# supersimple33/aruco-slam

Hardware: AMD Instinct MI355X
Metric: EKF updates/sec at n=1024 landmarks, m=32 obs/frame (higher is better)
Workload: dtype f32 covariance / f64 state

## Files before the change

aruco_slam_amd/csrc/ekf_api.hip:

```cpp
#include <atomic>
#include <cstring>

#include "ekf_host.h"
#include "ekf_kernels.h"

thread_local std::string g_err;

namespace {

std::atomic<ekf_filter*> g_pipelining{nullptr};

void release_pipelining_token(ekf_filter* f) { (void)g_pipelining.compare_exchange_strong(f, nullptr); }

constexpr int kStageSlots = 64;
constexpr int kMacroSuper = 8;
constexpr int kMacroMinTiles = 3000;
constexpr int kTimedKernels = 4;
constexpr int kWideVisible = 1024;
inline int visible_cap(int model) { return model == EKF_MODEL_ROTATIONS ? 50 : 64; }
inline bool wide_frame(int model, int m) { return m > visible_cap(model); }
constexpr int kEventPool = 2048;

struct Layout {
    int64_t cap;
// ... 39 lines not shown
    L.has_cov2 = c.cov_kernel != EKF_COVK_VALU && (c.flags & 5) == 0;
    L.off_cov2 = L.has_cov2 ? w.take((size_t)L.cap * L.cap * L.elem) : 0;
    L.off_wdbg = w.take((size_t)L.kmax * L.cap * 8);
    L.off_idx = w.take((size_t)c.max_visible * 4);
    L.off_z = w.take((size_t)c.max_visible * 7 * 8);
    L.off_status = w.take(256);
    L.off_stamps = w.take(64 * 8);
    L.off_dx = w.take((size_t)L.cap * 8);
    L.off_diag = w.take((size_t)L.cap * 8);
    L.off_xyz = w.take((size_t)256 * 6 * 8);
    L.off_unc = w.take((size_t)256 * 10 * 8);
    {
        const size_t nb = (size_t)L.kmax / EKF_RB;
        L.xl_dop = nb * (nb - 1) / 2 * 256 + 64;
        L.xl_y = L.xl_dop + nb * 256;
        L.xl_jac = L.xl_y + L.kmax;
        L.xl_tag = L.xl_jac + (size_t)L.kmax * EKF_JLD;
        L.xl_xs = L.xl_tag + 32;
        L.xl_xr = L.xl_xs + nb * (nb + 1) / 2 * 256;
        L.xl_stag = L.xl_xr + (size_t)round_up(L.kmax, 16);
        L.xl_len = L.xl_stag + 256;
        L.off_xl = w.take(2 * L.xl_len * 8);
        L.off_done = w.take(256);
        L.off_sync = w.take(256);
        L.wsup_ld = (int)round_up(EKF_CAM + (int64_t)L.lmd * c.max_visible, 32);
        L.off_wsup = w.take((size_t)2 * L.kmax * L.wsup_ld * L.elem);
    }
    {
        const int tmax = (int)(L.cap / 128);
        L.tiles_cap = (L.elem == 4 && c.cov_kernel != EKF_COVK_VALU && c.cov_kernel != EKF_COVK_MFMA_TILE)
                          ? tmax * (tmax + 1) / 2 + 8 * kMacroSuper * kMacroSuper : 0;
        L.off_tiles = w.take((size_t)L.tiles_cap * 4);
    }
    L.off_wwork = wide ? w.take((size_t)L.kmax * L.cap * 8) : 0;
    L.off_xinv = wide ? w.take((size_t)EKF_WIDE_BLOCK * EKF_WIDE_BLOCK * 8) : 0;
    L.total = w.end;
    L.slot_bytes = std::max(align256((size_t)c.max_visible * 4) + align256((size_t)c.max_visible * 56),
                            align256(256 * 48) + align256(256 * 80));
    return L;
}

int check_config(const ekf_config* c) {
    if (!c) return fail(EKF_ERR_INVALID, "config is NULL");
    if (c->max_landmarks < 1) return fail(EKF_ERR_INVALID, "max_landmarks must be >= 1");
    if (c->model != EKF_MODEL_EKF && c->model != EKF_MODEL_ROTATIONS)
        return fail(EKF_ERR_INVALID, "unknown model");
    if (c->max_visible < 1 || c->max_visible > ((c->flags & EKF_FLAG_WIDE_FRAMES) ? kWideVisible : visible_cap(c->model)))
// ... 109 lines not shown
    fr.idx = idx_dev;
    fr.z = z_dev;
    fr.jac = f->at<double>(L.off_jac);
    fr.resid = f->at<double>(L.off_resid);
    fr.lmcol = f->at<int32_t>(L.off_lmcol);
    fr.amat = f->at<double>(L.off_amat);
    fr.lda = L.cap;
    fr.sblk = f->at<double>(L.off_sblk);
    fr.sblk_rows = L.kmax;
    fr.lmat = f->at<double>(L.off_lmat);
    fr.ldl = L.kmax;
    fr.dinv = f->at<double>(L.off_dinv);
    fr.lop = f->at<double>(L.off_lop);
    fr.dop = f->at<double>(L.off_dop);
    fr.yvec = f->at<double>(L.off_y);
    fr.wpanel = f->at<void>(L.off_wpanel);
    fr.ldw = L.cap;
    fr.wdbg = f->debug_w ? f->at<double>(L.off_wdbg) : nullptr;
    fr.status = f->at<int32_t>(L.off_status);
    fr.traj_row = traj_row;
    fr.dxvec = f->at<double>(L.off_dx);
    fr.stamps = (f->debug_w || f->debug_stamps) ? f->at<long long>(L.off_stamps) : nullptr;
    fr.stamps_heavy = f->debug_stamps_light ? 0 : 1;
    fr.nz = EkfNoise{f->cfg.q_cam, f->cfg.q_err, f->cfg.q_lm, f->cfg.r_uncertainty};
    fr.quat_mode = f->cfg.quat_mode;
    fr.n_lm = f->n_lm;
    fr.state_host = nullptr;
    fr.status_host = nullptr;
    fr.cov_tiles = nullptr;
    fr.cov_grid = 0;
    if (f->tiles_T > 0 && f->tiles_T == (fr.dims + 127) / 128) {
        fr.cov_tiles = f->at<uint32_t>(L.off_tiles);
        fr.cov_grid = f->tiles_grid;
    }
    return fr;
}

bool use_front_kernel(const ekf_filter* f, const EkfFrame& fr) { return (f->cfg.flags & 4) == 0 && fr.kpad <= 192; }

void bind_exchange(ekf_filter* f, EkfFrame& fr) {
    const Layout& L = f->lay;
    double* base = f->at<double>(L.off_xl);
    fr.xl = base + (f->fseq & 1) * L.xl_len;
    fr.xl_next = base + ((f->fseq + 1) & 1) * L.xl_len;
    fr.xl_dop = (int32_t)L.xl_dop;
    fr.xl_y = (int32_t)L.xl_y;
// ... 237 lines not shown
            fr.wprev = wbuf[par ^ 1];
            fr.wsup_prev = wsup[par ^ 1];
        }
        const int nb = fr.kpad / EKF_RB;
        const int grid = nb * (nb + 1) / 2 + 2 + fr.ncols / 64;
        fr.wsup_ld = L.wsup_ld;
        fr.la_sync = sync;
        fr.la_signal = (t > 0) ? base + (uint64_t)t : 0;
        fr.la_gate = (t > 0) ? base + (uint64_t)t : 0;
        fr.lds_min = grid <= 100 ? 148 * 1024 : 0;
        if (t + 1 < frames) {
            nx = frame_at(t + 1);
            fr.next_idx = nx.idx;
            fr.next_m = nx.m;
            fr.wsup = wsup[par];
        }
        bind_exchange(f, fr);
        by_cov_type(f, [&](auto elem) { ekf_launch_front<decltype(elem)>(fr, f->stream); });
        EkfFrame cu = fr;
        cu.cov = cbuf[par];
        cu.cov_out = cbuf[par ^ 1];
        if (t + 1 < frames) {
            ekf_launch_gate(sync, base + (uint64_t)t + 1, status, f->big);
            by_cov_type(f, [&](auto elem) { ekf_launch_cov_update<decltype(elem)>(cu, 2, f->big); });
            ekf_launch_signal(sync + 1, base + (uint64_t)t + 1, f->big);
        } else {
            by_cov_type(f, [&](auto elem) { ekf_launch_cov_update<decltype(elem)>(cu, 2, f->stream); });
        }
        HIP_TRY(hipGetLastError());
        f->last_m = cf_t.m;
    }
    f->cov = cbuf[frames & 1];
    f->la_base = base + (uint64_t)frames;
    return EKF_OK;
}

struct RunPlan {
    std::vector<char> candidate;
    std::vector<char> joins;
    bool want_runs = false;
};

template <class MOf, class NNewOf>
RunPlan plan_runs(const ekf_filter* f, int frames, MOf m_of, NNewOf nnew_of) {
    RunPlan p;
    p.candidate.assign((size_t)frames, 0);
    p.joins.assign((size_t)frames, 0);
    int prev_kpad = -1;
// ... 689 lines not shown
            if (count < (size_t)kp * kp) return fail(EKF_ERR_INVALID, "out too small");
            HIP_TRY(hipMemcpy2D(out, (size_t)kp * 8, f->at<double>(L.off_lmat), (size_t)L.kmax * 8,
                                (size_t)kp * 8, kp, hipMemcpyDeviceToHost));
            return EKF_OK;
        case 3:
            if (!f->debug_w) return fail(EKF_ERR_STATE, "call ekf_debug_fetch(f,-1,..) first");
            if (count < (size_t)kp * dims) return fail(EKF_ERR_INVALID, "out too small");
            HIP_TRY(hipMemcpy2D(out, (size_t)dims * 8, f->at<double>(L.off_wdbg), (size_t)L.cap * 8,
                                (size_t)dims * 8, kp, hipMemcpyDeviceToHost));
            return EKF_OK;
        case 4:
            if (count < (size_t)k * dims) return fail(EKF_ERR_INVALID, "out too small");
            HIP_TRY(hipMemcpy2D(out, (size_t)dims * 8, f->at<double>(L.off_amat), (size_t)L.cap * 8,
                                (size_t)dims * 8, k, hipMemcpyDeviceToHost));
            return EKF_OK;
        case 5:
            if (count < 64) return fail(EKF_ERR_INVALID, "out too small");
            {
                long long st[64];
                HIP_TRY(hipMemcpy(st, f->at<long long>(L.off_stamps), sizeof(st), hipMemcpyDeviceToHost));
                for (int i = 0; i < 64; ++i) out[i] = (double)st[i];
            }
            return EKF_OK;
        default:
            return fail(EKF_ERR_INVALID, "unknown debug item");
    }
}

}
```

aruco_slam_amd/csrc/ekf_cov_macro.hip:

```cpp
#include <hip/hip_ext.h>
#include "ekf_kernels.h"

typedef float cm_f32x16 __attribute__((ext_vector_type(16)));
typedef float cm_f4 __attribute__((ext_vector_type(4)));

#define CM_NW 8
#define CM_T (64 * CM_NW)
#define CM_LD 132
#define CM_KC 16
#define CM_NBUF 5
#define CM_LDS_BYTES (CM_NBUF * 2 * CM_KC * 128 * 4)

#define CM_MID 0
#define CM_STAGGER 24000

__device__ __forceinline__ void cm_store16(float* p, const cm_f4& v) {
    asm volatile("global_store_dwordx4 %0, %1, off sc1\n\ts_nop 1" ::"v"(p), "v"(v) : "memory");
}

__device__ __forceinline__ void cm_dma16(const float* g, float* lds_wave_base) {
    __builtin_amdgcn_global_load_lds((const __attribute__((address_space(1))) void*)g,
                                     (__attribute__((address_space(3))) void*)lds_wave_base, 16, 0, 0);
}

// ... 13 lines not shown
        if (ch == target) seen = true;
    }
    for (int i = 0; i < steps; ++i) {
        if (i + depth < nch) {
            if (seen) n += dpw;
            if (i + depth == target) seen = true;
        }
        if (i < npb && seen) n += 16;
    }
    return n;
}
template <int N> __device__ __forceinline__ void cm_wait_vm() { asm volatile("s_waitcnt vmcnt(%0)" ::"n"(N) : "memory"); }

template <int KB, int NW>
__global__ __launch_bounds__(64 * NW) __attribute__((amdgpu_waves_per_eu(NW / 2, NW / 2)))
void ekf_cov_update_macro_f32(EkfFrame fr, const uint32_t* __restrict__ tiles) {
    extern __shared__ __attribute__((aligned(16))) float cm_sm[];
    constexpr int NT = 64 * NW, WC = NW / 2, CW = 128 / WC, TJ = CW / 32;
    constexpr int DPW = 16 / NW;
    constexpr int NPB = 2 * TJ;
    constexpr int DEPTH = CM_NBUF - 1;
    static_assert(NW == 8, "wait counts below are worked out for 8 waves");
    const uint32_t tl = tiles[blockIdx.x];
    if (tl == 0xFFFFFFFFu) return;
    const int I = (int)(tl >> 16), J = (int)(tl & 0xFFFFu);
    const int tid = threadIdx.x, lane = tid & 63, l31 = lane & 31, lhi = lane >> 5;
    const int wave = __builtin_amdgcn_readfirstlane(tid >> 6);
    const int wr = wave / WC, wc = wave % WC;
    const int i0 = 128 * I, j0 = 128 * J;
    const float* __restrict__ wp = static_cast<const float*>(fr.wpanel);
    const float* __restrict__ P = static_cast<const float*>(fr.cov);
    float* Pout = fr.cov_out ? static_cast<float*>(fr.cov_out) : static_cast<float*>(fr.cov);
    const int ld = (int)fr.ld, ldw = (int)fr.ldw;
    constexpr int NCH = KB;

    if (blockIdx.x < 512 && ((__builtin_amdgcn_s_getreg((31 << 11) | 4) / (NW / 4)) & 1)) {
        const long long t0 = __builtin_amdgcn_s_memtime();
        while (__builtin_amdgcn_s_memtime() - t0 < CM_STAGGER) __builtin_amdgcn_s_sleep(32);
    }
    const unsigned wlane = (unsigned)(lhi * ldw + 4 * l31);
    auto stage = [&](int c) {
        float* buf = cm_sm + (c % CM_NBUF) * (2 * CM_KC * 128);
        const int rloc = 2 * wave;
        const float* src = wp + (int64_t)(CM_KC * c + rloc) * ldw;
        cm_dma16(src + i0 + wlane, buf + rloc * 128);
        cm_dma16(src + j0 + wlane, buf + CM_KC * 128 + rloc * 128);
    };
// ... 107 lines not shown
        for (int it = 0; it < NPASS; ++it) cm_store16(ob + (int64_t)(RPP * it) * ld + (unsigned)(prow * ld + pcol), rowv[it]);
    }
    if (!dtile) __syncthreads();
    if (!dtile) {
#pragma unroll
    for (int ti = 0; ti < 2; ++ti)
#pragma unroll
        for (int tj = 0; tj < TJ; ++tj)
#pragma unroll
            for (int rg = 0; rg < 4; ++rg) {
                const cm_f4 v = {acc[ti][tj][4 * rg], acc[ti][tj][4 * rg + 1], acc[ti][tj][4 * rg + 2], acc[ti][tj][4 * rg + 3]};
                *reinterpret_cast<cm_f4*>(img + (CW * wc + 32 * tj + l31) * CM_LD + 64 * wr + 32 * ti + 8 * rg + 4 * lhi) = v;
            }
    __syncthreads();
    {
        cm_f4 rowv[NPASS];
#pragma unroll
        for (int it = 0; it < NPASS; ++it) rowv[it] = *reinterpret_cast<const cm_f4*>(img + (RPP * it + prow) * CM_LD + pcol);
        float* ob = Pout + (int64_t)j0 * ld + i0;
#pragma unroll
        for (int it = 0; it < NPASS; ++it) cm_store16(ob + (int64_t)(RPP * it) * ld + (unsigned)(prow * ld + pcol), rowv[it]);
    }
    }
}

int ekf_cov_macro_table(int T, int S, uint32_t* out, int capacity) {
    struct Sup { int si, sj, count; };
    const int NS = (T + S - 1) / S;
    Sup sup[4096];
    int nsup = 0;
    for (int si = 0; si < NS; ++si)
        for (int sj = 0; sj <= si; ++sj) {
            int cnt = 0;
            for (int I = si * S; I < T && I < (si + 1) * S; ++I)
                for (int J = sj * S; J < T && J < (sj + 1) * S && J <= I; ++J) ++cnt;
            if (cnt > 0 && nsup < 4096) sup[nsup++] = Sup{si, sj, cnt};
        }
    for (int a = 1; a < nsup; ++a) {
        const Sup x = sup[a];
        int b = a - 1;
        while (b >= 0 && sup[b].count < x.count) { sup[b + 1] = sup[b]; --b; }
        sup[b + 1] = x;
    }
    int load[8] = {0, 0, 0, 0, 0, 0, 0, 0};
    int owner[4096];
    for (int a = 0; a < nsup; ++a) {
// ... 45 lines not shown
```

aruco_slam_amd/csrc/ekf_cov_update.hip:

```cpp
#include <hip/hip_ext.h>
#include "ekf_kernels.h"

template <typename T>
__device__ __forceinline__ void ekf_cov_store(T* p, T v) {
    __hip_atomic_store(p, v, __ATOMIC_RELAXED, __HIP_MEMORY_SCOPE_AGENT);
}

typedef float f32x16 __attribute__((ext_vector_type(16)));
typedef double f64x4 __attribute__((ext_vector_type(4)));

template <typename T>
__global__ __launch_bounds__(256) void ekf_cov_update_valu(EkfFrame fr) {
    __shared__ T sa[16][64];
    __shared__ T sb[16][64];
    const int tid = threadIdx.x, tx = tid & 15, ty = tid >> 4;
    const int i0 = blockIdx.y * 64, j0 = blockIdx.x * 64;
    const T* __restrict__ wp = static_cast<const T*>(fr.wpanel);
    T acc[4][4];
#pragma unroll
    for (int x = 0; x < 4; ++x)
#pragma unroll
        for (int y = 0; y < 4; ++y) acc[x][y] = (T)0;
    for (int kc = 0; kc < fr.kpad; kc += 16) {
#pragma unroll
// ... 26 lines not shown
            const int col = j0 + tx * 4 + y;
            T v = P[(int64_t)row * fr.ld + col];
            if (row == col) v += (T)ekf_qdiag(row, fr.dims, fr.nz);
            P[(int64_t)row * fr.ld + col] = v + acc[x][y];
        }
    }
}

__device__ __forceinline__ void ekf_tri_decode(int item, int& I, int& J) {
    int i = (int)((sqrtf(8.0f * (float)item + 1.0f) - 1.0f) * 0.5f);
    while (i * (i + 1) / 2 > item) --i;
    while ((i + 1) * (i + 2) / 2 <= item) ++i;
    I = i;
    J = item - i * (i + 1) / 2;
}

template <int KB, int DMAX = 3, int WPE = 5>
__global__ __launch_bounds__(256) __attribute__((amdgpu_waves_per_eu(WPE, WPE)))
void ekf_cov_update_mfma_f32(EkfFrame fr, int nitems) {
    __shared__ float tr[4][32][33];
    const int wave = threadIdx.x >> 6, lane = threadIdx.x & 63;
    const int l31 = lane & 31, lhi = lane >> 5;
    const int item = __builtin_amdgcn_readfirstlane(blockIdx.x * 4 + wave);
    if (item >= nitems) return;
    int I, J;
    ekf_tri_decode(item, I, J);
    const int i0 = 32 * I, j0 = 32 * J;
    const float* __restrict__ wp = static_cast<const float*>(fr.wpanel);
    const float* __restrict__ P = static_cast<const float*>(fr.cov);
    float* Pout = fr.cov_out ? static_cast<float*>(fr.cov_out) : static_cast<float*>(fr.cov);
    const int ld = (int)fr.ld, ldw = (int)fr.ldw;
    constexpr int NCH = KB, D = (NCH < DMAX) ? NCH : DMAX;
    float ra[D][8], rb[D][8], pt[16];
    const unsigned wlane = 4u * (unsigned)(lhi * ldw + l31);
    const unsigned plane = 4u * (unsigned)(4 * lhi * ld + l31);
    const uint64_t kstep = 8ull * (uint64_t)ldw;
    uint64_t ua = reinterpret_cast<uint64_t>(wp + i0), ub = reinterpret_cast<uint64_t>(wp + j0);
    const float* __restrict__ ptile = P + (int64_t)i0 * ld + j0;
    float* otile = Pout + (int64_t)i0 * ld + j0;
#define EKF_GLD(dst, voff, sbase) asm volatile("global_load_dword %0, %1, %2" : "=v"(dst) : "v"(voff), "s"(sbase) : "memory")
#define EKF_WAIT16(n, A, B)                                                                              \
    asm volatile("s_waitcnt vmcnt(%16)"                                                                   \
                 : "+v"(A[0]), "+v"(A[1]), "+v"(A[2]), "+v"(A[3]), "+v"(A[4]), "+v"(A[5]), "+v"(A[6]), "+v"(A[7]), \
                   "+v"(B[0]), "+v"(B[1]), "+v"(B[2]), "+v"(B[3]), "+v"(B[4]), "+v"(B[5]), "+v"(B[6]), "+v"(B[7])  \
                 : "n"(n))
    f32x16 acc;
#pragma unroll
// ... 49 lines not shown
#undef EKF_GLD
#undef EKF_WAIT16
    const float qlane = (I == J) ? (float)ekf_qdiag(i0 + l31, fr.dims, fr.nz) : 0.0f;
    float out[16];
    auto stf = [](float* base, unsigned off, float v) { ekf_cov_store(reinterpret_cast<float*>(reinterpret_cast<char*>(base) + off), v); };
#pragma unroll
    for (int reg = 0; reg < 16; ++reg) {
        const int rl = (reg & 3) + 8 * (reg >> 2) + 4 * lhi;
        const float v = (pt[reg] + ((rl == l31) ? qlane : 0.0f)) + acc[reg];
        out[reg] = v;
        stf(otile + (int64_t)((reg & 3) + 8 * (reg >> 2)) * ld, plane, v);
    }
    if (I != J) {
#pragma unroll
        for (int reg = 0; reg < 16; ++reg)
            tr[wave][(reg & 3) + 8 * (reg >> 2) + 4 * lhi][l31] = out[reg];
        __builtin_amdgcn_wave_barrier();
        float* pm = Pout + (int64_t)j0 * ld + i0;
        const unsigned mlane = 4u * (unsigned)(lhi * ld + l31);
#pragma unroll
        for (int it = 0; it < 16; ++it)
            stf(pm + (int64_t)(2 * it) * ld, mlane, tr[wave][l31][2 * it + lhi]);
    }
}

__global__ __launch_bounds__(256) void ekf_cov_update_mfma_f64(EkfFrame fr, int nitems) {
    __shared__ double tr[4][32][33];
    const int wave = threadIdx.x >> 6, lane = threadIdx.x & 63;
    const int c = lane & 15, g = lane >> 4;
    const int item = blockIdx.x * 4 + wave;
    if (item >= nitems) return;
    int I, J;
    ekf_tri_decode(item, I, J);
    const int i0 = 32 * I, j0 = 32 * J;
    const double* __restrict__ wp = static_cast<const double*>(fr.wpanel);
    const double* P = static_cast<const double*>(fr.cov);
    double* Pout = fr.cov_out ? static_cast<double*>(fr.cov_out) : static_cast<double*>(fr.cov);
    const int64_t ld = fr.ld, ldw = fr.ldw;

    double pt[2][2][4];
#pragma unroll
    for (int ri = 0; ri < 2; ++ri)
#pragma unroll
        for (int ci = 0; ci < 2; ++ci)
#pragma unroll
            for (int r = 0; r < 4; ++r)
                pt[ri][ci][r] = P[(int64_t)(i0 + 16 * ri + g + 4 * r) * ld + j0 + 16 * ci + c];
    f64x4 acc[2][2];
#pragma unroll
    for (int ri = 0; ri < 2; ++ri)
#pragma unroll
        for (int ci = 0; ci < 2; ++ci)
#pragma unroll
            for (int r = 0; r < 4; ++r) acc[ri][ci][r] = 0.0;
// ... 20 lines not shown
    }
#pragma unroll
    for (int ri = 0; ri < 2; ++ri)
#pragma unroll
        for (int ci = 0; ci < 2; ++ci)
#pragma unroll
            for (int r = 0; r < 4; ++r) {
                const int rl = 16 * ri + g + 4 * r, cl = 16 * ci + c;
                double v = pt[ri][ci][r];
                if (I == J && rl == cl) v += ekf_qdiag(i0 + rl, fr.dims, fr.nz);
                v += acc[ri][ci][r];
                ekf_cov_store(Pout + (int64_t)(i0 + rl) * ld + j0 + cl, v);
                if (I != J) tr[wave][rl][cl] = v;
            }
    if (I != J) {
        __builtin_amdgcn_wave_barrier();
        const int l31 = lane & 31, lhi = lane >> 5;
#pragma unroll
        for (int it = 0; it < 16; ++it) {
            const int cc = 2 * it + lhi;
            ekf_cov_store(Pout + (int64_t)(j0 + cc) * ld + i0 + l31, tr[wave][l31][cc]);
        }
    }
}

__global__ __launch_bounds__(256) void ekf_cov_update_mfma_f64_split(EkfFrame fr, int nitems) {
    __shared__ double tr[32][33];
    const int wave = threadIdx.x >> 6, lane = threadIdx.x & 63;
    const int c = lane & 15, g = lane >> 4;
    const int ri = wave >> 1, ci = wave & 1;
    int I, J;
    ekf_tri_decode(blockIdx.x, I, J);
    const int i0 = 32 * I, j0 = 32 * J;
    const double* __restrict__ wp = static_cast<const double*>(fr.wpanel);
    const double* P = static_cast<const double*>(fr.cov);
    double* Pout = fr.cov_out ? static_cast<double*>(fr.cov_out) : static_cast<double*>(fr.cov);
    const int64_t ld = fr.ld, ldw = fr.ldw;
    double pt[4];
#pragma unroll
    for (int r = 0; r < 4; ++r) pt[r] = P[(int64_t)(i0 + 16 * ri + g + 4 * r) * ld + j0 + 16 * ci + c];
    f64x4 acc = {0.0, 0.0, 0.0, 0.0};
    const double* wa = wp + (int64_t)g * ldw + i0 + 16 * ri + c;
    const double* wb = wp + (int64_t)g * ldw + j0 + 16 * ci + c;
    const int steps = fr.kpad >> 2;
    for (int ks = 0; ks < steps; ks += 4) {
        double a[4], b[4];
// ... 1 lines not shown
        for (int u = 0; u < 4; ++u) {
            const int64_t off = (int64_t)(4 * (ks + u)) * ldw;
            a[u] = wa[off];
            b[u] = wb[off];
        }
#pragma unroll
        for (int u = 0; u < 4; ++u) acc = __builtin_amdgcn_mfma_f64_16x16x4f64(-a[u], b[u], acc, 0, 0, 0);
    }
#pragma unroll
    for (int r = 0; r < 4; ++r) {
        const int rl = 16 * ri + g + 4 * r, cl = 16 * ci + c;
        double v = pt[r];
        if (I == J && rl == cl) v += ekf_qdiag(i0 + rl, fr.dims, fr.nz);
        v += acc[r];
        ekf_cov_store(Pout + (int64_t)(i0 + rl) * ld + j0 + cl, v);
        if (I != J) tr[rl][cl] = v;
    }
    if (I != J) {
        __syncthreads();
        const int l31 = threadIdx.x & 31;
        for (int cc = threadIdx.x >> 5; cc < 32; cc += 8)
            ekf_cov_store(Pout + (int64_t)(j0 + cc) * ld + i0 + l31, tr[l31][cc]);
    }
}

__global__ void ekf_gate_kernel(unsigned long long* counter, unsigned long long target, int32_t* status, int max_polls) {
    if (threadIdx.x != 0) return;
    int it = 0;
    while (__hip_atomic_load(counter, __ATOMIC_RELAXED, __HIP_MEMORY_SCOPE_SYSTEM) < target) {
        if (++it > max_polls) { atomicOr(status, EKF_ST_GATE_TIMEOUT); break; }
        __builtin_amdgcn_s_sleep(8);
    }
}
__global__ void ekf_signal_kernel(unsigned long long* counter, unsigned long long value) {
    if (threadIdx.x == 0) __hip_atomic_store(counter, value, __ATOMIC_RELAXED, __HIP_MEMORY_SCOPE_SYSTEM);
}
void ekf_launch_gate(unsigned long long* counter, unsigned long long target, int32_t* status, hipStream_t s, int max_polls) {
    hipLaunchKernelGGL(ekf_gate_kernel, dim3(1), dim3(64), 0, s, counter, target, status, max_polls);
}
void ekf_launch_signal(unsigned long long* counter, unsigned long long value, hipStream_t s) {
    hipLaunchKernelGGL(ekf_signal_kernel, dim3(1), dim3(64), 0, s, counter, value);
}

#define EKF_COV_LAUNCH(kernel, grid, block, s, e0, e1, ...)                                     \
    do {                                                                                         \
        if (e0) hipExtLaunchKernelGGL(kernel, grid, block, 0, s, e0, e1, 0, __VA_ARGS__);        \
// ... 41 lines not shown
```

aruco_slam_amd/csrc/ekf_front_impl.h:

```cpp
#pragma once
#include "ekf_solve_big.h"

#define FR_T 512
#define FR_ALD 66
#define FR_KS 96
#define FR_KS64 48
__host__ __device__ inline size_t fr_chunk_a_len(int kpad, bool fix, int elem) {
    const size_t a = (size_t)kpad * FR_ALD;
    const size_t st = elem == 4 ? (size_t)(FR_KS * 128 + FR_KS * 64 + 128 * 64) / 2 : (size_t)(2 * FR_KS64 * 64 + 64 * 64);
    return (fix && a < st) ? st : a;
}
#define FR_SLOTS 4

typedef double pf64x4 __attribute__((ext_vector_type(4)));
template <typename T>
__device__ __forceinline__ void fr_w_store(T* p, T v) {
    __hip_atomic_store(p, v, __ATOMIC_RELAXED, __HIP_MEMORY_SCOPE_AGENT);
}
typedef float fr_f32x16 __attribute__((ext_vector_type(16)));

__device__ __forceinline__ void ekf_poll_sleep() { __builtin_amdgcn_s_sleep(4); }

template <int MODEL>
__device__ __forceinline__ void fr_measure(const EkfFrame& fr, const double* cam, const int* lmc, double* hs,
// ... 191 lines not shown
    __syncthreads();
    if (tid < 256) us[(tid >> 4) * 17 + (tid & 15)] = v;
    __syncthreads();
    if (tid < 64) {
        sv_sblock_emit<true>(fr.xs + sv_blk_index(bi, bj), us, bi == bj, tid);
        if (tid == 0) ekf_stc(fr.xs_tag + 16 * bj + bi, fr.seqno);
    }
    if (fr.stamps && sb == nS - 1 && tid == 0) fr.stamps[61] = wall_clock64();

    {
        const int64_t lo = (int64_t)fr.xl_len * sb / nS, hi = (int64_t)fr.xl_len * (sb + 1) / nS;
        const double sent = ekf_sent();
        for (int64_t e = lo + tid; e < hi; e += FR_T) ekf_stc(fr.xl_next + e, sent);
    }
}

template <int MODEL>
__device__ __forceinline__ void fr_role_measure(const EkfFrame& fr, double* sm) {
    constexpr int LMD = EkfModel<MODEL>::LMD, JC = EkfModel<MODEL>::JC;
    double* hs = sm;
    double* rsd = sm + fr.k * JC;
    int* lmc = reinterpret_cast<int*>(rsd + fr.kpad);
    const int tid = threadIdx.x;
    if (fr.stamps && !fr.stamps_heavy && tid == 0) fr.stamps[16 + ((long long)fr.seqno & 15)] = wall_clock64();
    if (fr.la_signal && tid == 0)
        __hip_atomic_store(fr.la_sync, fr.la_signal, __ATOMIC_RELAXED, __HIP_MEMORY_SCOPE_SYSTEM);
    double cam[EKF_CAM];
#pragma unroll
    for (int a = 0; a < EKF_CAM; ++a) cam[a] = fr.state[a];
    if (tid < fr.m) lmc[tid] = ekf_lm_column(fr, LMD, tid, true);
    __syncthreads();
    fr_measure<MODEL>(fr, cam, lmc, hs, rsd, tid, true);
    __syncthreads();
    double* __restrict__ xj = fr.xl + fr.xl_jac;
    const int nel = fr.k * JC;
    for (int e = tid; e < nel; e += FR_T) ekf_stc(xj + e, hs[e]);
    for (int e = tid; e < fr.kpad; e += FR_T) ekf_stc(fr.xr + e, rsd[e]);
    if (tid == 0) {
        ekf_stc(fr.xl + fr.xl_tag, fr.seqno);
        ekf_stc(fr.xl + fr.xl_tag + 16, fr.seqno);
    }
    if (fr.stamps && tid == 0) fr.stamps[55] = wall_clock64();
    if (fr.la_gate && tid == 0) {
        int it = 0;
        while (__hip_atomic_load(fr.la_sync + 1, __ATOMIC_RELAXED, __HIP_MEMORY_SCOPE_SYSTEM) < fr.la_gate) {
            if (++it > (1 << 22)) { ekf_raise(fr, EKF_ST_GATE_TIMEOUT); break; }
            __builtin_amdgcn_s_sleep(8);
        }
    }
}

__device__ __forceinline__ int fr_tag_stale(double tag, double seqno) { return !ekf_is_sent(tag) && tag != seqno; }
struct SvIoFused {
    const EkfFrame& fr;
    int spin_fail, stale;
    __device__ __forceinline__ bool settled(const sf64x4& v) const {
        return !__any(ekf_is_sent(v[0]) || ekf_is_sent(v[1]) || ekf_is_sent(v[2]) || ekf_is_sent(v[3]));
    }
    __device__ __forceinline__ void settle_block(sf64x4& v, int i, int tc, int lane) {
        const double* base = fr.xs + sv_blk_index(i, tc);
        int it = 0;
        while (!settled(v)) {
            if (++it > EKF_SPIN_MAX) { spin_fail = 1; break; }
            ekf_poll_sleep();
            v = sf64x4{ekf_ldc(base + 2 * lane), ekf_ldc(base + 2 * lane + 1), ekf_ldc(base + 128 + 2 * lane),
                       ekf_ldc(base + 129 + 2 * lane)};
        }
    }
    __device__ __forceinline__ sf64x4 fetch_resid(int tc, int g) {
        const double* base = fr.xr + EKF_RB * tc + g;
// ... 866 lines not shown
```

aruco_slam_amd/csrc/ekf_kernels.h:

```cpp
#pragma once
#include <hip/hip_runtime.h>
#include <stdint.h>
#include "ekf_device.h"

#define EKF_ST_NOT_SPD 1
#define EKF_ST_TIMEOUT 4
#define EKF_ST_STALE_JAC 16
#define EKF_ST_STALE_COL 32
#define EKF_ST_STALE_S 64
#define EKF_ST_BAD_INDEX 128
#define EKF_ST_GATE_TIMEOUT 256

struct EkfFrame {
    void* cov;
    int64_t ld;
    double* state;
    int32_t model;
    int32_t dims;
    int32_t ncols;
    int32_t m;
    int32_t k;
    int32_t kpad;
    const int32_t* idx;
    const double* z;
// ... 5 lines not shown
    double* sblk;
    int32_t sblk_rows;
    double* lmat;
    int32_t ldl;
    double* dinv;
    double* lop;
    double* dop;
    double* yvec;
    void* wpanel;
    int64_t ldw;
    double* wdbg;
    int32_t* status;
    double* traj_row;
    double* dxvec;
    long long* stamps;
    int32_t stamps_heavy;
    const int32_t* next_idx;
    int32_t next_m;
    void* cov_out;
    const void* wprev;
    const void* wsup_prev;
    unsigned long long* la_sync;
    unsigned long long la_signal, la_gate;
    int32_t lds_min;
    void* wsup;
    int32_t wsup_ld;
    EkfNoise nz;
    int32_t quat_mode;
    double* xl;
    double* xl_next;
    int32_t xl_dop, xl_y, xl_jac;
    int32_t xl_len;
    double* xs;
    double* xr;
    double* xs_tag;
    int32_t n_lm;
    unsigned long long* done_ctr;
    unsigned long long done_target;
    int32_t xl_tag;
    double seqno;
    double* state_host;
    int32_t* status_host;
    const uint32_t* cov_tiles;
    int32_t cov_grid;
};

__device__ __forceinline__ void ekf_raise(const EkfFrame& fr, int bits) {
    atomicOr(fr.status, bits);
    if (fr.status_host) __hip_atomic_store(fr.status_host, 1, __ATOMIC_RELAXED, __HIP_MEMORY_SCOPE_SYSTEM);
}

__device__ __forceinline__ int ekf_lm_column(const EkfFrame& fr, int lmd, int j, bool flag) {
    int i = fr.idx[j];
    if ((unsigned)i >= (unsigned)fr.n_lm) {
        if (flag) ekf_raise(fr, EKF_ST_BAD_INDEX);
        i = 0;
    }
    return EKF_CAM + lmd * i;
}

__device__ inline void ekf_inject_camera(const EkfFrame& fr, const double err[3], const double x[3]) {
    double q[4] = {fr.state[3], fr.state[4], fr.state[5], fr.state[6]};
    ekf_quat_inject(q, err, fr.quat_mode);
    for (int i = 0; i < 4; ++i) fr.state[3 + i] = q[i];
    for (int i = 0; i < 3; ++i) fr.state[7 + i] = 0.0;
    if (fr.traj_row) {
        fr.traj_row[0] = x[0]; fr.traj_row[1] = x[1]; fr.traj_row[2] = x[2];
        for (int i = 0; i < 4; ++i) fr.traj_row[3 + i] = q[i];
    }
}

template <typename T> void ekf_launch_front(const EkfFrame& fr, hipStream_t s);
// ... 86 lines not shown
```

aruco_slam_amd/csrc/ekf_solve_cw.h:

```cpp
#pragma once
#include <type_traits>
#include "ekf_solve_device.h"

#define SVC_WORKERS 6

__host__ __device__ constexpr int svc_lds_doubles(int nb) {
    return nb * 256 + (nb + 1) * nb * 256 + nb * 512 + (2 * nb + 2 + 1) / 2 + 8;
}

__device__ __forceinline__ bool svc_wait_ok(volatile ekf_lds_int* word, int want) {
    int it = 0;
    bool ok = true;
    while (*word < want) {
        if (++it > (1 << 22)) { ok = false; break; }
        __builtin_amdgcn_s_sleep(1);
    }
    __builtin_amdgcn_fence(__ATOMIC_ACQUIRE, "workgroup");
    return ok;
}
__device__ __forceinline__ void svc_post(volatile ekf_lds_int* word, int value, int lane) {
    __builtin_amdgcn_fence(__ATOMIC_RELEASE, "workgroup");
    if (lane == 0) *word = value;
}
__device__ __forceinline__ void svc_post_in_order(volatile ekf_lds_int* word, int value, int lane) {
    asm volatile("" ::: "memory");
    if (lane == 0) *word = value;
    asm volatile("" ::: "memory");
}

template <int B0, int N, class F>
__device__ __forceinline__ void svc_static_for(F&& f) {
    if constexpr (B0 < N) {
        if (f(std::integral_constant<int, B0>{})) svc_static_for<B0 + 1, N>(f);
    }
}

template <int NB, class IO>
__device__ __forceinline__ void sv_factor_cw(const EkfFrame& fr, IO& io, double* lds, int& bad, int& badcol) {
    static_assert(NB >= 1 && NB <= 6, "block columns");
    const int tid = threadIdx.x, lane = tid & 63, c = lane & 15, g = lane >> 4;
    const int wave = __builtin_amdgcn_readfirstlane(tid >> 6);
    double* xbuf = lds;
    double* ybuf = xbuf + NB * 256;
    double* dep = ybuf + (NB + 1) * NB * 256;
    volatile ekf_lds_int* xready = ekf_lds_flags(dep + NB * 512);
    volatile ekf_lds_int* yflag = xready + 1;
    volatile ekf_lds_int* dready = yflag + (NB + 1);
    for (int e = tid; e < 2 * NB + 2; e += SV_T) xready[e] = 0;
    __syncthreads();
    const bool is_chain = wave == 0, is_pub = wave == 4;
    auto svc_wait = [&](volatile ekf_lds_int* word, int want) {
        if (!svc_wait_ok(word, want)) {
            if (!bad) badcol = 200 + (int)(word - xready);
            bad = 1;
        }
    };
    auto yb = [&](int i, int b) { return ybuf + ((size_t)i * NB + b) * 256; };
    long long* stl = (fr.stamps && !fr.stamps_heavy && is_pub && lane == 0) ? fr.stamps : nullptr;
    if (stl) stl[0] = clock64();

    if (is_chain) {
        {
            sf64x4 idm;
#pragma unroll
            for (int r = 0; r < 4; ++r) idm[r] = (g + 4 * r == c) ? 1.0 : 0.0;
            const SvChainRes warm = sv_chain_shared(idm, lane);
            asm volatile("" ::"v"(warm.xop[0]), "v"(warm.bad));
        }
        svc_wait(dready, 1);
        sf64x4 d = sv_lds_get(dep + 256, lane);
#pragma unroll
// ... 3 lines not shown
            if (fr.wdbg) {
                SvChain s;
                s.m = d;
                badnow = sv_chain_t<true>(s, xop, c, g);
#pragma unroll
                for (int r = 0; r < 4; ++r) {
                    const int col = g + 4 * r;
                    const double sq = s.dr[r] * ekf_rsqrt_f64(s.dr[r]);
                    fr.lmat[(size_t)(EKF_RB * b + c) * fr.ldl + EKF_RB * b + col] = (c >= col) ? s.lp[r] * sq : 0.0;
                }
            } else {
                const SvChainRes res = sv_chain_shared(d, lane);
                xop = res.xop;
                badnow = res.bad;
            }
            if (badnow && !bad) badcol = 100 + b;
            bad |= badnow;
            sf64x4 p = {0.0, 0.0, 0.0, 0.0};
            if (b + 1 < NB) {
                svc_wait(dready + (b + 1), 1);
                p = sv_lds_get(dep + (b + 1) * 512, lane);
                d = sv_lds_get(dep + (b + 1) * 512 + 256, lane);
            }
            sv_lds_put(xbuf + b * 256, xop, lane);
            svc_post_in_order(xready, b + 1, lane);
            if (b + 1 < NB) {
                const sf64x4 y = sv_mm(xop, p);
                sv_mm_sub(d, y, y);
                sv_lds_put(yb(b + 1, b), y, lane);
                svc_post_in_order(yflag + (b + 1), b + 1, lane);
                if (fr.wdbg) {
#pragma unroll
                    for (int r = 0; r < 4; ++r) fr.lmat[(size_t)(EKF_RB * (b + 1) + c) * fr.ldl + EKF_RB * b + g + 4 * r] = y[r];
                }
            }
        }
        return;
    }
    if (is_pub) {
#pragma unroll
        for (int b = 0; b < NB; ++b) {
            svc_wait(xready, b + 1);
            if (stl) stl[2 + 2 * b] = clock64();
            io.put_dinv(b, sv_lds_get(xbuf + b * 256, lane), lane);
#pragma unroll
            for (int i = b + 1; i <= NB; ++i) {
                svc_wait(yflag + i, b + 1);
                const sf64x4 yi = sv_lds_get(yb(i, b), lane);
                if (i < NB) io.put_l(i, b, yi, lane);
                else io.put_y(b, (c >> 2) == 0 ? yi[0] : (c >> 2) == 1 ? yi[1] : (c >> 2) == 2 ? yi[2] : yi[3], c, g == (c & 3));
            }
        }
        return;
    }
    const int widx = wave < 4 ? wave - 1 : wave - 2;
    const int i0 = widx, i1 = widx + SVC_WORKERS;
    const bool has0 = i0 <= NB, has1 = i1 <= NB;
    sf64x4 z0[NB], z1[NB];
    io.template load_cols<NB, NB, NB, 0, 1>(z0, z1, i0, i1, has0, has1, lane, g);
    if (has0 && i0 == 0) {
        sv_lds_put(dep + 256, z0[0], lane);
        svc_post(dready, 1, lane);
    }
    if (NB > 1) io.template load_cols<NB, NB, NB, 1, NB>(z0, z1, i0, i1, has0, has1, lane, g);
    if (NB > 1 && has0 && i0 == 1) {
        sv_lds_put(dep + 512, z0[0], lane);
        sv_lds_put(dep + 512 + 256, z0[1], lane);
        svc_post(dready + 1, 1, lane);
    }
    auto row_step = [&](sf64x4 (&z)[NB], int i, auto bc, const sf64x4& xop) {
        constexpr int b = decltype(bc)::value;
        if (i <= b) return;
        if (i == b + 1 && i < NB) return;
        const sf64x4 y = sv_mm(xop, z[b]);
        sv_lds_put(yb(i, b), y, lane);
        svc_post(yflag + i, b + 1, lane);
        if (fr.wdbg && i < NB) {
#pragma unroll
            for (int r = 0; r < 4; ++r) fr.lmat[(size_t)(EKF_RB * i + c) * fr.ldl + EKF_RB * b + g + 4 * r] = y[r];
        }
        svc_static_for<b + 1, NB>([&](auto tcc) {
            constexpr int tc = decltype(tcc)::value;
            if (tc > i) return false;
            if (tc == i) sv_mm_sub(z[tc], y, y);
            else {
                svc_wait(yflag + tc, b + 1);
                sv_mm_sub(z[tc], sv_lds_get(yb(tc, b), lane), y);
            }
            if constexpr (tc == b + 2) {
                if (i == tc) {
                    sv_lds_put(dep + i * 512, z[b + 1], lane);
                    sv_lds_put(dep + i * 512 + 256, z[b + 2], lane);
                    svc_post(dready + i, 1, lane);
                }
            }
            return true;
        });
    };
    svc_static_for<0, NB>([&](auto bc) {
        constexpr int b = decltype(bc)::value;
        if (!((has0 && i0 > b) || (has1 && i1 > b))) return false;
        svc_wait(xready, b + 1);
        const sf64x4 xop = sv_lds_get(xbuf + b * 256, lane);
        if (has0) row_step(z0, i0, bc, xop);
        if (has1) row_step(z1, i1, bc, xop);
        return true;
    });
}
```

aruco_slam_amd/hip_backend.py:

```python
from __future__ import annotations

import ctypes as C
from pathlib import Path

import numpy as np

from ._build import LIB_PATH

EKF_COV_F64, EKF_COV_F32 = 0, 1
EKF_QUAT_AS_WRITTEN, EKF_QUAT_SCALAR_FIRST = 0, 1
EKF_FLAG_WIDE_FRAMES = 8
EKF_FLAG_BATCH_LARGE_MAPS = 16
EKF_FLAG_BATCH_WIDE_FRAMES = 32
EKF_COVK_AUTO, EKF_COVK_VALU, EKF_COVK_MFMA, EKF_COVK_MFMA_TILE, EKF_COVK_MFMA_MACRO = 0, 1, 2, 3, 4

EXPORTED_SYMBOLS = (
    "ekf_default_config", "ekf_query_sizes", "ekf_create", "ekf_destroy", "ekf_bind_buffers",
    "ekf_reset", "ekf_grow", "ekf_add_markers", "ekf_observe", "ekf_observe_device",
    "ekf_observe_sequence_device", "ekf_last_sequence_mode", "ekf_get_camera", "ekf_get_state", "ekf_get_cov_diag",
    "ekf_get_cov", "ekf_set_state", "ekf_set_cov", "ekf_num_landmarks", "ekf_sync",
    "ekf_set_fused", "ekf_set_kernel_timing", "ekf_get_kernel_timing", "ekf_debug_fetch",
    "ekf_estimate_poses_device", "ekf_estimate_poses", "ekf_last_error_string",
    "ekf_log_workspace_bytes", "ekf_observe_log", "ekf_last_log_stats",
    "ekf_batch_query_sizes", "ekf_batch_create", "ekf_batch_bind_buffers", "ekf_batch_destroy", "ekf_batch_set_noise",
    "ekf_batch_reset", "ekf_batch_set_member", "ekf_batch_get_member", "ekf_batch_num_landmarks", "ekf_batch_status",
    "ekf_batch_log_workspace_bytes", "ekf_batch_observe_logs", "ekf_batch_observe_logs_diag", "ekf_batch_replica_poses",
    "ekf_batch_replica_workspace_bytes", "ekf_batch_observe_replicas",
    "ekf_batch_set_gate", "ekf_batch_observe_logs_gated", "ekf_batch_observe_replicas_gated",
)


class EkfConfig(C.Structure):
    _fields_ = [
        ("max_landmarks", C.c_int32), ("max_visible", C.c_int32), ("cov_dtype", C.c_int32),
        ("quat_mode", C.c_int32), ("cov_kernel", C.c_int32), ("model", C.c_int32), ("reserved", C.c_int32), ("flags", C.c_int32),
        ("initial_camera_uncertainty", C.c_double), ("initial_landmark_uncertainty", C.c_double),
        ("r_uncertainty", C.c_double), ("q_cam", C.c_double), ("q_err", C.c_double),
# ... 342 lines not shown
            out = {"front": out["gather"], "cov_update": out["cov_update"]}
        return out

    def set_fused(self, enable: bool):
        self._check(self.lib.ekf_set_fused(self.h, int(bool(enable))))
        if enable:
            self.cfg.flags &= ~4
        else:
            self.cfg.flags |= 4
        self.fused = bool(enable)

    def debug_enable_w(self):
        dummy = np.zeros(1)
        self._check(self.lib.ekf_debug_fetch(self.h, -1, _dptr(dummy), 1))

    def debug_enable_stamps(self, light: bool = False):
        dummy = np.zeros(1)
        self._check(self.lib.ekf_debug_fetch(self.h, -3 if light else -2, _dptr(dummy), 1))

    def debug_fetch(self, what: str, m: int):
        rd = self.rows_per_detection
        k, kp, n = rd * m, -(-rd * m // 16) * 16, self.dims
        shape = {"jac": (k, 20 if rd == 7 else 13), "resid": (k,), "L": (kp, kp), "W": (kp, n), "A": (k, n),
                 "stamps": (64,)}[what]
        code = {"jac": 0, "resid": 1, "L": 2, "W": 3, "A": 4, "stamps": 5}[what]
        out = np.empty(shape)
        self._check(self.lib.ekf_debug_fetch(self.h, code, _dptr(out), out.size))
        return out
```

Measured before the change: 42690.

## Signal cov-update completion from the kernel tail, shorten the solve chain

Removes the separate signal kernel after each covariance update. Each cov-update block now arrives on a sharded atomic counter when it finishes, and the last arriver publishes the frame's completion word, so the next frame's front kernel can pass its gate sooner. The triangular solve also lets the chain wave finish the last block's dinv and y output directly from a dedicated LDS slot, instead of handing it to the publisher wave. A debug gate-wait log is added as well. In exchange every block pays a vmcnt wait, a barrier and atomics at its tail.

```diff
diff --git a/aruco_slam_amd/csrc/ekf_api.hip b/aruco_slam_amd/csrc/ekf_api.hip
--- a/aruco_slam_amd/csrc/ekf_api.hip
+++ b/aruco_slam_amd/csrc/ekf_api.hip
@@ -85,7 +85,7 @@
         L.xl_len = L.xl_stag + 256;
         L.off_xl = w.take(2 * L.xl_len * 8);
         L.off_done = w.take(256);
-        L.off_sync = w.take(256);
+        L.off_sync = w.take(EKF_SYNC_WORDS * 8);
         L.wsup_ld = (int)round_up(EKF_CAM + (int64_t)L.lmd * c.max_visible, 32);
         L.off_wsup = w.take((size_t)2 * L.kmax * L.wsup_ld * L.elem);
     }
@@ -241,6 +241,8 @@
     fr.dxvec = f->at<double>(L.off_dx);
     fr.stamps = (f->debug_w || f->debug_stamps) ? f->at<long long>(L.off_stamps) : nullptr;
     fr.stamps_heavy = f->debug_stamps_light ? 0 : 1;
+    fr.gate_log = (fr.stamps && !fr.stamps_heavy && !f->debug_w && (size_t)L.kmax * L.cap >= 4 * EKF_GATE_LOG_FRAMES)
+                      ? f->at<long long>(L.off_wdbg) : nullptr;
     fr.nz = EkfNoise{f->cfg.q_cam, f->cfg.q_err, f->cfg.q_lm, f->cfg.r_uncertainty};
     fr.quat_mode = f->cfg.quat_mode;
     fr.n_lm = f->n_lm;
@@ -524,8 +526,8 @@
         cu.cov_out = cbuf[par ^ 1];
         if (t + 1 < frames) {
             ekf_launch_gate(sync, base + (uint64_t)t + 1, status, f->big);
+            cu.cov_signal = base + (uint64_t)t + 1;
             by_cov_type(f, [&](auto elem) { ekf_launch_cov_update<decltype(elem)>(cu, 2, f->big); });
-            ekf_launch_signal(sync + 1, base + (uint64_t)t + 1, f->big);
         } else {
             by_cov_type(f, [&](auto elem) { ekf_launch_cov_update<decltype(elem)>(cu, 2, f->stream); });
         }
@@ -1261,6 +1263,16 @@
                 for (int i = 0; i < 64; ++i) out[i] = (double)st[i];
             }
             return EKF_OK;
+        case 6:
+            if (count < 4 * EKF_GATE_LOG_FRAMES) return fail(EKF_ERR_INVALID, "out too small");
+            if (!(f->debug_stamps && f->debug_stamps_light) || f->debug_w || (size_t)L.kmax * L.cap < 4 * EKF_GATE_LOG_FRAMES)
+                return fail(EKF_ERR_STATE, "the gate log needs role-level stamps (ekf_debug_fetch(f,-3,..)) and kmax * cap >= 8192");
+            {
+                std::vector<long long> st(4 * EKF_GATE_LOG_FRAMES);
+                HIP_TRY(hipMemcpy(st.data(), f->at<long long>(L.off_wdbg), st.size() * 8, hipMemcpyDeviceToHost));
+                for (size_t i = 0; i < st.size(); ++i) out[i] = (double)st[i];
+            }
+            return EKF_OK;
         default:
             return fail(EKF_ERR_INVALID, "unknown debug item");
     }
diff --git a/aruco_slam_amd/csrc/ekf_cov_macro.hip b/aruco_slam_amd/csrc/ekf_cov_macro.hip
--- a/aruco_slam_amd/csrc/ekf_cov_macro.hip
+++ b/aruco_slam_amd/csrc/ekf_cov_macro.hip
@@ -59,7 +59,10 @@
     constexpr int DEPTH = CM_NBUF - 1;
     static_assert(NW == 8, "wait counts below are worked out for 8 waves");
     const uint32_t tl = tiles[blockIdx.x];
-    if (tl == 0xFFFFFFFFu) return;
+    if (tl == 0xFFFFFFFFu) {
+        if (fr.cov_signal) ekf_cov_arrive(fr);
+        return;
+    }
     const int I = (int)(tl >> 16), J = (int)(tl & 0xFFFFu);
     const int tid = threadIdx.x, lane = tid & 63, l31 = lane & 31, lhi = lane >> 5;
     const int wave = __builtin_amdgcn_readfirstlane(tid >> 6);
@@ -213,6 +216,7 @@
         for (int it = 0; it < NPASS; ++it) cm_store16(ob + (int64_t)(RPP * it) * ld + (unsigned)(prow * ld + pcol), rowv[it]);
     }
     }
+    if (fr.cov_signal) ekf_cov_arrive(fr);
 }
 
 int ekf_cov_macro_table(int T, int S, uint32_t* out, int capacity) {
diff --git a/aruco_slam_amd/csrc/ekf_cov_update.hip b/aruco_slam_amd/csrc/ekf_cov_update.hip
--- a/aruco_slam_amd/csrc/ekf_cov_update.hip
+++ b/aruco_slam_amd/csrc/ekf_cov_update.hip
@@ -72,7 +72,10 @@
     const int wave = threadIdx.x >> 6, lane = threadIdx.x & 63;
     const int l31 = lane & 31, lhi = lane >> 5;
     const int item = __builtin_amdgcn_readfirstlane(blockIdx.x * 4 + wave);
-    if (item >= nitems) return;
+    if (item >= nitems) {
+        if (fr.cov_signal) ekf_cov_arrive(fr);
+        return;
+    }
     int I, J;
     ekf_tri_decode(item, I, J);
     const int i0 = 32 * I, j0 = 32 * J;
@@ -168,6 +171,7 @@
         for (int it = 0; it < 16; ++it)
             stf(pm + (int64_t)(2 * it) * ld, mlane, tr[wave][l31][2 * it + lhi]);
     }
+    if (fr.cov_signal) ekf_cov_arrive(fr);
 }
 
 __global__ __launch_bounds__(256) void ekf_cov_update_mfma_f64(EkfFrame fr, int nitems) {
@@ -175,7 +179,10 @@
     const int wave = threadIdx.x >> 6, lane = threadIdx.x & 63;
     const int c = lane & 15, g = lane >> 4;
     const int item = blockIdx.x * 4 + wave;
-    if (item >= nitems) return;
+    if (item >= nitems) {
+        if (fr.cov_signal) ekf_cov_arrive(fr);
+        return;
+    }
     int I, J;
     ekf_tri_decode(item, I, J);
     const int i0 = 32 * I, j0 = 32 * J;
@@ -242,6 +249,7 @@
             ekf_cov_store(Pout + (int64_t)(j0 + cc) * ld + i0 + l31, tr[wave][l31][cc]);
         }
     }
+    if (fr.cov_signal) ekf_cov_arrive(fr);
 }
 
 __global__ __launch_bounds__(256) void ekf_cov_update_mfma_f64_split(EkfFrame fr, int nitems) {
@@ -289,6 +297,7 @@
         for (int cc = threadIdx.x >> 5; cc < 32; cc += 8)
             ekf_cov_store(Pout + (int64_t)(j0 + cc) * ld + i0 + l31, tr[l31][cc]);
     }
+    if (fr.cov_signal) ekf_cov_arrive(fr);
 }
 
 __global__ void ekf_gate_kernel(unsigned long long* counter, unsigned long long target, int32_t* status, int max_polls) {
diff --git a/aruco_slam_amd/csrc/ekf_front_impl.h b/aruco_slam_amd/csrc/ekf_front_impl.h
--- a/aruco_slam_amd/csrc/ekf_front_impl.h
+++ b/aruco_slam_amd/csrc/ekf_front_impl.h
@@ -237,7 +237,11 @@
     double* rsd = sm + fr.k * JC;
     int* lmc = reinterpret_cast<int*>(rsd + fr.kpad);
     const int tid = threadIdx.x;
-    if (fr.stamps && !fr.stamps_heavy && tid == 0) fr.stamps[16 + ((long long)fr.seqno & 15)] = wall_clock64();
+    if (fr.stamps && !fr.stamps_heavy && tid == 0) {
+        const long long now = wall_clock64();
+        fr.stamps[16 + ((long long)fr.seqno & 15)] = now;
+        if (fr.gate_log) fr.gate_log[4 * ((long long)fr.seqno & (EKF_GATE_LOG_FRAMES - 1))] = now;
+    }
     if (fr.la_signal && tid == 0)
         __hip_atomic_store(fr.la_sync, fr.la_signal, __ATOMIC_RELAXED, __HIP_MEMORY_SCOPE_SYSTEM);
     double cam[EKF_CAM];
@@ -257,10 +261,17 @@
     }
     if (fr.stamps && tid == 0) fr.stamps[55] = wall_clock64();
     if (fr.la_gate && tid == 0) {
+        const long long g0 = fr.gate_log ? wall_clock64() : 0;
         int it = 0;
         while (__hip_atomic_load(fr.la_sync + 1, __ATOMIC_RELAXED, __HIP_MEMORY_SCOPE_SYSTEM) < fr.la_gate) {
             if (++it > (1 << 22)) { ekf_raise(fr, EKF_ST_GATE_TIMEOUT); break; }
             __builtin_amdgcn_s_sleep(8);
+        }
+        if (fr.gate_log) {
+            long long* row = fr.gate_log + 4 * ((long long)fr.seqno & (EKF_GATE_LOG_FRAMES - 1));
+            row[1] = g0;
+            row[2] = wall_clock64();
+            row[3] = it;
         }
     }
 }
diff --git a/aruco_slam_amd/csrc/ekf_kernels.h b/aruco_slam_amd/csrc/ekf_kernels.h
--- a/aruco_slam_amd/csrc/ekf_kernels.h
+++ b/aruco_slam_amd/csrc/ekf_kernels.h
@@ -51,6 +51,8 @@
     const void* wsup_prev;
     unsigned long long* la_sync;
     unsigned long long la_signal, la_gate;
+    unsigned long long cov_signal;
+    long long* gate_log;
     int32_t lds_min;
     void* wsup;
     int32_t wsup_ld;
@@ -77,6 +79,28 @@
 __device__ __forceinline__ void ekf_raise(const EkfFrame& fr, int bits) {
     atomicOr(fr.status, bits);
     if (fr.status_host) __hip_atomic_store(fr.status_host, 1, __ATOMIC_RELAXED, __HIP_MEMORY_SCOPE_SYSTEM);
+}
+
+#define EKF_COV_SHARDS 8
+#define EKF_SYNC_SHARD(s) (32 + 32 * (s))
+#define EKF_SYNC_WORDS EKF_SYNC_SHARD(EKF_COV_SHARDS + 1)
+#define EKF_GATE_LOG_FRAMES 2048
+__device__ __forceinline__ bool ekf_cov_count(unsigned long long* ctr, unsigned long long full) {
+    if (__hip_atomic_fetch_add(ctr, 1ull, __ATOMIC_RELAXED, __HIP_MEMORY_SCOPE_AGENT) + 1 != full) return false;
+    __hip_atomic_store(ctr, 0ull, __ATOMIC_RELAXED, __HIP_MEMORY_SCOPE_AGENT);
+    return true;
+}
+__device__ __forceinline__ void ekf_cov_arrive(const EkfFrame& fr) {
+    asm volatile("s_waitcnt vmcnt(0)" ::: "memory");
+    __builtin_amdgcn_s_barrier();
+    if (threadIdx.x == 0) {
+        const unsigned grid = gridDim.x, sh = blockIdx.x % EKF_COV_SHARDS;
+        const unsigned in_shard = (grid + EKF_COV_SHARDS - 1 - sh) / EKF_COV_SHARDS;
+        const unsigned shards = grid < EKF_COV_SHARDS ? grid : EKF_COV_SHARDS;
+        if (ekf_cov_count(fr.la_sync + EKF_SYNC_SHARD(sh), in_shard) &&
+            ekf_cov_count(fr.la_sync + EKF_SYNC_SHARD(EKF_COV_SHARDS), shards))
+            __hip_atomic_store(fr.la_sync + 1, fr.cov_signal, __ATOMIC_RELAXED, __HIP_MEMORY_SCOPE_SYSTEM);
+    }
 }
 
 __device__ __forceinline__ int ekf_lm_column(const EkfFrame& fr, int lmd, int j, bool flag) {
diff --git a/aruco_slam_amd/csrc/ekf_solve_cw.h b/aruco_slam_amd/csrc/ekf_solve_cw.h
--- a/aruco_slam_amd/csrc/ekf_solve_cw.h
+++ b/aruco_slam_amd/csrc/ekf_solve_cw.h
@@ -5,7 +5,7 @@
 #define SVC_WORKERS 6
 
 __host__ __device__ constexpr int svc_lds_doubles(int nb) {
-    return nb * 256 + (nb + 1) * nb * 256 + nb * 512 + (2 * nb + 2 + 1) / 2 + 8;
+    return nb * 256 + (nb + 1) * nb * 256 + nb * 512 + 256 + (2 * nb + 3 + 1) / 2 + 8;
 }
 
 __device__ __forceinline__ bool svc_wait_ok(volatile ekf_lds_int* word, int want) {
@@ -43,10 +43,12 @@
     double* xbuf = lds;
     double* ybuf = xbuf + NB * 256;
     double* dep = ybuf + (NB + 1) * NB * 256;
-    volatile ekf_lds_int* xready = ekf_lds_flags(dep + NB * 512);
+    double* rlast = dep + NB * 512;
+    volatile ekf_lds_int* xready = ekf_lds_flags(rlast + 256);
     volatile ekf_lds_int* yflag = xready + 1;
     volatile ekf_lds_int* dready = yflag + (NB + 1);
-    for (int e = tid; e < 2 * NB + 2; e += SV_T) xready[e] = 0;
+    volatile ekf_lds_int* rready = dready + NB;
+    for (int e = tid; e < 2 * NB + 3; e += SV_T) xready[e] = 0;
     __syncthreads();
     const bool is_chain = wave == 0, is_pub = wave == 4;
     auto svc_wait = [&](volatile ekf_lds_int* word, int want) {
@@ -96,6 +98,14 @@
                 p = sv_lds_get(dep + (b + 1) * 512, lane);
                 d = sv_lds_get(dep + (b + 1) * 512 + 256, lane);
             }
+            if (b + 1 == NB) {
+                io.put_dinv(b, xop, lane);
+                svc_wait(rready, 1);
+                const sf64x4 yi = sv_mm(xop, sv_lds_get(rlast, lane));
+                io.put_y(b, (c >> 2) == 0 ? yi[0] : (c >> 2) == 1 ? yi[1] : (c >> 2) == 2 ? yi[2] : yi[3], c, g == (c & 3));
+                if (fr.stamps && !fr.stamps_heavy && lane == 0) fr.stamps[1] = clock64();
+                break;
+            }
             sv_lds_put(xbuf + b * 256, xop, lane);
             svc_post_in_order(xready, b + 1, lane);
             if (b + 1 < NB) {
@@ -113,7 +123,7 @@
     }
     if (is_pub) {
 #pragma unroll
-        for (int b = 0; b < NB; ++b) {
+        for (int b = 0; b + 1 < NB; ++b) {
             svc_wait(xready, b + 1);
             if (stl) stl[2 + 2 * b] = clock64();
             io.put_dinv(b, sv_lds_get(xbuf + b * 256, lane), lane);
@@ -136,6 +146,10 @@
         sv_lds_put(dep + 256, z0[0], lane);
         svc_post(dready, 1, lane);
     }
+    if (NB == 1 && has0 && i0 == 1) {
+        sv_lds_put(rlast, z0[0], lane);
+        svc_post(rready, 1, lane);
+    }
     if (NB > 1) io.template load_cols<NB, NB, NB, 1, NB>(z0, z1, i0, i1, has0, has1, lane, g);
     if (NB > 1 && has0 && i0 == 1) {
         sv_lds_put(dep + 512, z0[0], lane);
@@ -170,8 +184,14 @@
             }
             return true;
         });
+        if constexpr (b + 2 == NB) {
+            if (i == NB) {
+                sv_lds_put(rlast, z[NB - 1], lane);
+                svc_post(rready, 1, lane);
+            }
+        }
     };
-    svc_static_for<0, NB>([&](auto bc) {
+    svc_static_for<0, NB - 1>([&](auto bc) {
         constexpr int b = decltype(bc)::value;
         if (!((has0 && i0 > b) || (has1 && i1 > b))) return false;
         svc_wait(xready, b + 1);
diff --git a/aruco_slam_amd/hip_backend.py b/aruco_slam_amd/hip_backend.py
--- a/aruco_slam_amd/hip_backend.py
+++ b/aruco_slam_amd/hip_backend.py
@@ -13,6 +13,8 @@
 EKF_FLAG_BATCH_LARGE_MAPS = 16
 EKF_FLAG_BATCH_WIDE_FRAMES = 32
 EKF_COVK_AUTO, EKF_COVK_VALU, EKF_COVK_MFMA, EKF_COVK_MFMA_TILE, EKF_COVK_MFMA_MACRO = 0, 1, 2, 3, 4
+
+GATE_LOG_FRAMES = 2048
 
 EXPORTED_SYMBOLS = (
     "ekf_default_config", "ekf_query_sizes", "ekf_create", "ekf_destroy", "ekf_bind_buffers",
@@ -401,8 +403,8 @@
         rd = self.rows_per_detection
         k, kp, n = rd * m, -(-rd * m // 16) * 16, self.dims
         shape = {"jac": (k, 20 if rd == 7 else 13), "resid": (k,), "L": (kp, kp), "W": (kp, n), "A": (k, n),
-                 "stamps": (64,)}[what]
-        code = {"jac": 0, "resid": 1, "L": 2, "W": 3, "A": 4, "stamps": 5}[what]
+                 "stamps": (64,), "gate_log": (GATE_LOG_FRAMES, 4)}[what]
+        code = {"jac": 0, "resid": 1, "L": 2, "W": 3, "A": 4, "stamps": 5, "gate_log": 6}[what]
         out = np.empty(shape)
         self._check(self.lib.ekf_debug_fetch(self.h, code, _dptr(out), out.size))
         return out
```

Result: faster. 43310 (median of 6 runs) (+1.5%).
